# Chrissie-Law/Causal-Domain-Clustering-for-Multi-Domain-Recommendation

Hardware: AMD Instinct MI355X
Metric: train samples/sec + AUC parity, PLE 3-domain batch 4096 at 1/2/4/8 MI355X (higher is better)
Workload: dtype bf16; 1 GPU; PLE 3-domain full training step (fwd + BCE + whole-table L2 + bwd + Adam), 26 fields x vocab 1000000, emb_dim=16, batch 4096/GPU; global_batch=4096, table_mode=lazy, hip_graph=True, row_sort_one_batch_ahead=True, id_dist=uniform, parallelism=dp1, attention_branch=False, full=False, steady_state=True, preroll_steps=1785, flush_every=64

## Files before the change

causal-domain-clustering-for-multi-domain-recommendation_amd/csrc/embedding.hip:

```cpp
#include "common.h"
#include "adam_dense.h"

template <int VEC>
__global__ void __launch_bounds__(256) k_gather_fwd(const int32_t* __restrict__ ids, const int32_t* __restrict__ offsets,
                                                    const float* __restrict__ table, float* __restrict__ out,
                                                    __bf16* __restrict__ out_h, int64_t ld_out_h,
                                                    int32_t* __restrict__ idx_out, int32_t* __restrict__ err_flag,
                                                    int64_t n_pos, int32_t F, int32_t D, int64_t R) {
    CDC_PRIO_MAIN();
    const int chunks = D / VEC;
    const int64_t total = n_pos * chunks;
    for (int64_t i = (int64_t)blockIdx.x * blockDim.x + threadIdx.x; i < total; i += (int64_t)gridDim.x * blockDim.x) {
        const int64_t pos = i / chunks;
        const int c = (int)(i - pos * chunks);
        const int f = (int)(pos % F);
        const int32_t row = (int32_t)((uint32_t)ids[pos] + (uint32_t)offsets[f]);
        const bool ok = row >= 0 && (int64_t)row < R;
        if (c == 0 && idx_out) idx_out[pos] = ok ? row : -1;
        if (!ok && c == 0 && err_flag) atomicMax(err_flag, (int32_t)(pos < 0x7ffffffe ? pos + 1 : 0x7fffffff));
        if (VEC == 4) {
            float4 val = make_float4(0.f, 0.f, 0.f, 0.f);
            if (ok) val = *reinterpret_cast<const float4*>(table + (int64_t)row * D + c * 4);
            *reinterpret_cast<float4*>(out + pos * D + c * 4) = val;
            if (out_h) {
                typedef __bf16 h4_t __attribute__((ext_vector_type(4)));
                h4_t h = {(__bf16)val.x, (__bf16)val.y, (__bf16)val.z, (__bf16)val.w};
                *reinterpret_cast<h4_t*>(out_h + (pos / F) * ld_out_h + (int64_t)f * D + c * 4) = h;
            }
        } else {
            const float v = ok ? table[(int64_t)row * D + c] : 0.f;
            out[pos * D + c] = v;
            if (out_h) out_h[(pos / F) * ld_out_h + (int64_t)f * D + c] = (__bf16)v;
        }
    }
}

extern "C" int cdc_embed_gather_fwd(const int32_t* ids, const int32_t* offsets, const float* table, float* out,
                                    int32_t* idx_out, int32_t* err_flag, int64_t B, int32_t F, int32_t D, int64_t R,
                                    void* stream) {
    return cdc_embed_gather_fwd_h(ids, offsets, table, out, nullptr, 0, idx_out, err_flag, B, F, D, R, stream);
}
extern "C" int cdc_embed_gather_fwd_h(const int32_t* ids, const int32_t* offsets, const float* table, float* out, void* out_h_,
                                      int64_t ld_out_h, int32_t* idx_out, int32_t* err_flag, int64_t B, int32_t F, int32_t D, int64_t R,
                                      void* stream) {
    __bf16* out_h = reinterpret_cast<__bf16*>(out_h_);
    CDC_CHECK_ARG(ids && offsets && table && out, CDC_E_BADARG, "embed_gather_fwd: null pointer");
    CDC_CHECK_ARG(!out_h || (ld_out_h >= (int64_t)F * D && (((uintptr_t)out_h) & 7) == 0 && ld_out_h % 4 == 0), CDC_E_BADARG,
                  "embed_gather_fwd: malformed bf16 shadow");
    CDC_CHECK_ARG(B >= 0 && F > 0 && D > 0 && R > 0, CDC_E_BADARG, "embed_gather_fwd: bad sizes B=%ld F=%d D=%d R=%ld",
                  (long)B, F, D, (long)R);
    if (B == 0) return 0;
    const int64_t n_pos = B * F;
    const bool vec = (D % 4 == 0) && (((uintptr_t)table | (uintptr_t)out) % 16 == 0);
    const int64_t total = n_pos * (vec ? D / 4 : D);
    int blocks = (int)std::min<int64_t>(cdc_ceil_div(total, 256), 256 * 16);
    if (vec)
        hipLaunchKernelGGL(k_gather_fwd<4>, dim3(blocks), dim3(256), 0, (hipStream_t)stream, ids, offsets, table, out, out_h, ld_out_h,
                           idx_out, err_flag, n_pos, F, D, R);
    else
        hipLaunchKernelGGL(k_gather_fwd<1>, dim3(blocks), dim3(256), 0, (hipStream_t)stream, ids, offsets, table, out, out_h, ld_out_h,
                           idx_out, err_flag, n_pos, F, D, R);
    CDC_LAUNCH_CHECK("embed_gather_fwd");
    return 0;
}

__global__ void __launch_bounds__(256) k_embed_index(const int32_t* __restrict__ ids, const int32_t* __restrict__ offsets,
                                                     int32_t* __restrict__ idx_out, int32_t* __restrict__ err_flag, int64_t n_pos,
                                                     int32_t F, int64_t R) {
    for (int64_t pos = (int64_t)blockIdx.x * blockDim.x + threadIdx.x; pos < n_pos; pos += (int64_t)gridDim.x * blockDim.x) {
        const int32_t row = (int32_t)((uint32_t)ids[pos] + (uint32_t)offsets[pos % F]);
        const bool ok = row >= 0 && (int64_t)row < R;
        if (!ok && err_flag) atomicMax(err_flag, (int32_t)(pos < 0x7ffffffe ? pos + 1 : 0x7fffffff));
        idx_out[pos] = ok ? row : -1;
    }
}
extern "C" int cdc_embed_index(const int32_t* ids, const int32_t* offsets, int32_t* idx_out, int32_t* err_flag, int64_t B, int32_t F,
                               int64_t R, void* stream) {
    CDC_CHECK_ARG(ids && offsets && idx_out && B > 0 && F > 0 && R > 0, CDC_E_BADARG, "embed_index: bad argument");
    int blocks = (int)std::min<int64_t>(cdc_ceil_div(B * F, 256), 4096);
    hipLaunchKernelGGL(k_embed_index, dim3(blocks), dim3(256), 0, (hipStream_t)stream, ids, offsets, idx_out, err_flag, B * F, F, R);
    CDC_LAUNCH_CHECK("embed_index");
    return 0;
}

#define SORT_THREADS 1024
#define SORT_CHUNK CDC_SORT_MAX_B

__device__ __forceinline__ void lds_bitonic_sort(uint64_t* keys, int n_pad, int tid) {
    for (int k = 2; k <= n_pad; k <<= 1) {
        for (int j = k >> 1; j > 0; j >>= 1) {
            for (int t = tid; t < (n_pad >> 1); t += SORT_THREADS) {
                const int lo = ((t & ~(j - 1)) << 1) | (t & (j - 1));
                const int hi = lo | j;
                const bool up = (lo & k) == 0;
                const uint64_t a = keys[lo], b = keys[hi];
                if ((a > b) == up) { keys[lo] = b; keys[hi] = a; }
            }
            const int next_j = j > 1 ? (j >> 1) : k;
            if (j >= 64 || next_j >= 64) __syncthreads();
            else {
                __builtin_amdgcn_fence(__ATOMIC_SEQ_CST, "wavefront");
                __builtin_amdgcn_wave_barrier();
            }
        }
    }
    __syncthreads();
}

__device__ __forceinline__ int block_exclusive_scan(int v, int32_t* wave_tot, int tid, int& total) {
    const int lane = tid & 63, wave = tid >> 6;
    int inc = v;
#pragma unroll
    for (int off = 1; off < 64; off <<= 1) {
        const int t = __shfl_up(inc, off, 64);
        if (lane >= off) inc += t;
    }
    if (lane == 63) wave_tot[wave] = inc;
    __syncthreads();
    int base = 0, all = 0;
#pragma unroll
    for (int w = 0; w < SORT_THREADS / 64; ++w) {
        const int t = wave_tot[w];
        base += (w < wave) ? t : 0;
        all += t;
    }
    __syncthreads();
    total = all;
    return base + inc - v;
}

__device__ __forceinline__ void dedupe_sorted(const uint64_t* keys, int n, int32_t* scan, int32_t* __restrict__ urow,
                                              int32_t* __restrict__ sst, int32_t* __restrict__ prm, int32_t* __restrict__ cnt_out,
                                              int tid) {
    const int per = (n + SORT_THREADS - 1) / SORT_THREADS;
    const int begin = tid * per;
    int local = 0;
    for (int i = begin; i < begin + per && i < n; ++i) {
        const bool head = (i == 0) || ((keys[i] >> 32) != (keys[i - 1] >> 32));
        local += head ? 1 : 0;
    }
    int total;
    int u = block_exclusive_scan(local, scan, tid, total);
    for (int i = begin; i < begin + per && i < n; ++i) {
        const uint64_t k = keys[i];
        const bool head = (i == 0) || ((k >> 32) != (keys[i - 1] >> 32));
        if (head) {
            urow[u] = (int32_t)(uint32_t)(k >> 32);
            sst[u] = i;
            ++u;
        }
        prm[i] = (int32_t)(uint32_t)k;
    }
    if (tid == 0) {
        sst[total] = n;
        *cnt_out = total;
    }
}

struct SortSrc {
    const int32_t* idx;
    const int32_t* offsets;
    int64_t R;
    int32_t* step;
    double* acc;
    int32_t n_acc;
    int32_t* err_flag;
};
__device__ __forceinline__ uint32_t sort_row(const SortSrc& s, int64_t i, int f, int F) {
    const int32_t v = s.idx[i * F + f];
    if (!s.offsets) return (uint32_t)v;
    const int32_t row = (int32_t)((uint32_t)v + (uint32_t)s.offsets[f]);
    if (row >= 0 && (int64_t)row < s.R) return (uint32_t)row;
    if (s.err_flag) {
        const int64_t pos = i * F + f;
        atomicMax(s.err_flag, (int32_t)(pos < 0x7ffffffe ? pos + 1 : 0x7fffffff));
    }
    return 0xffffffffu;
}
__device__ __forceinline__ void sort_begin_step(const SortSrc& s, int tid) {
    if (s.step && blockIdx.x == 0 && blockIdx.y == 0) {
        if (tid == 0) *s.step += 1;
        if (tid < s.n_acc) s.acc[tid] = 0.0;
    }
}

__global__ void __launch_bounds__(SORT_THREADS) k_sort_dedupe(const SortSrc src, int32_t* __restrict__ uniq_row,
                                                              int32_t* __restrict__ seg_start, int32_t* __restrict__ perm,
                                                              int32_t* __restrict__ uniq_cnt, int32_t B, int32_t F,
                                                              int32_t n_pad) {
    extern __shared__ __attribute__((aligned(16))) unsigned char smem_raw[];
    uint64_t* keys = reinterpret_cast<uint64_t*>(smem_raw);
    int32_t* scan = reinterpret_cast<int32_t*>(keys + n_pad);
    const int f = blockIdx.x;
    const int tid = threadIdx.x;
    for (int i = tid; i < n_pad; i += SORT_THREADS) {
        uint64_t k = ~0ull;
        if (i < B) k = ((uint64_t)sort_row(src, i, f, F) << 32) | (uint32_t)i;
        keys[i] = k;
    }
    sort_begin_step(src, tid);
    __syncthreads();
    lds_bitonic_sort(keys, n_pad, tid);
    dedupe_sorted(keys, B, scan, uniq_row + (int64_t)f * B, seg_start + (int64_t)f * (B + 1), perm + (int64_t)f * B, uniq_cnt + f, tid);
}

__global__ void __launch_bounds__(SORT_THREADS) k_sort_chunk(const SortSrc src, uint64_t* __restrict__ runs, int32_t B,
                                                             int32_t F, int32_t chunk) {
    extern __shared__ __attribute__((aligned(16))) unsigned char smem_raw[];
    uint64_t* keys = reinterpret_cast<uint64_t*>(smem_raw);
    const int f = blockIdx.x, c = blockIdx.y, tid = threadIdx.x;
    const int r0 = c * chunk;
    const int n = min(chunk, B - r0);
    for (int i = tid; i < chunk; i += SORT_THREADS) {
        uint64_t k = ~0ull;
        if (i < n) k = ((uint64_t)sort_row(src, r0 + i, f, F) << 32) | (uint32_t)(r0 + i);
        keys[i] = k;
    }
    sort_begin_step(src, tid);
    __syncthreads();
    lds_bitonic_sort(keys, chunk, tid);
    uint64_t* out = runs + (int64_t)f * B + r0;
    for (int i = tid; i < n; i += SORT_THREADS) out[i] = keys[i];
}
__device__ __forceinline__ int group_sum(int v, int P) {
    for (int off = 1; off < P; off <<= 1) v += __shfl_xor(v, off, 64);
    return v;
}
__global__ void __launch_bounds__(256) k_merge_runs(const uint64_t* __restrict__ runs, uint64_t* __restrict__ merged, int32_t B,
                                                    int32_t F, int32_t chunk, int32_t n_runs, int32_t P) {
    const int64_t t = (int64_t)blockIdx.x * blockDim.x + threadIdx.x;
    const int64_t item = t / P;
    const int q = (int)(t - item * P);
    const bool valid = item < (int64_t)F * B;
    const int f = valid ? (int)(item / B) : 0;
    const int i = valid ? (int)(item - (int64_t)f * B) : 0;
    const uint64_t* a = runs + (int64_t)f * B;
    const uint64_t key = a[i];
    const int r = i / chunk;
    int lo = 0;
    if (valid && q < n_runs) {
        if (q == r) lo = i - r * chunk;
        else {
            const uint64_t* other = a + (int64_t)q * chunk;
            int hi = min(chunk, B - q * chunk);
            while (lo < hi) {
                const int mid = (lo + hi) >> 1;
                if (other[mid] < key) lo = mid + 1; else hi = mid;
            }
        }
    }
    const int pos = group_sum(lo, P);
    if (valid && q == 0) merged[(int64_t)f * B + pos] = key;
}
template <typename K, bool IDX>
__global__ void __launch_bounds__(SORT_THREADS) k_merge_lds(const void* __restrict__ src, uint64_t* __restrict__ merged, int32_t B,
                                                            int32_t F, int32_t n_runs, int32_t run_len, int32_t P) {
    extern __shared__ __attribute__((aligned(16))) unsigned char smem_raw[];
    K* keys = reinterpret_cast<K*>(smem_raw);
    const int f = blockIdx.x, r = blockIdx.y, tid = threadIdx.x;
    if (IDX) {
        const int32_t* idx = static_cast<const int32_t*>(src);
        for (int i = tid; i < B; i += SORT_THREADS) keys[i] = (K)(uint32_t)idx[(int64_t)i * F + f];
    } else {
        const uint64_t* a = static_cast<const uint64_t*>(src) + (int64_t)f * B;
        for (int i = tid; i < B; i += SORT_THREADS) keys[i] = (K)a[i];
    }
    __syncthreads();
    const int base = r * run_len;
    const int n_r = min(run_len, B - base);
    const int rounds = (n_r * P + SORT_THREADS - 1) / SORT_THREADS;
    for (int it = 0; it < rounds; ++it) {
        const int t = it * SORT_THREADS + tid;
        const int item = t / P, q = t - item * P;
        const bool valid = item < n_r;
        const K key = keys[valid ? base + item : base];
        int lo = 0;
        if (valid && q < n_runs) {
            if (q == r) lo = item;
            else {
                const K* other = keys + q * run_len;
                int hi = min(run_len, B - q * run_len);
                if (IDX && q < r) { while (lo < hi) { const int mid = (lo + hi) >> 1; if (other[mid] <= key) lo = mid + 1; else hi = mid; } }
                else              { while (lo < hi) { const int mid = (lo + hi) >> 1; if (other[mid] <  key) lo = mid + 1; else hi = mid; } }
            }
        }
        const int pos = group_sum(lo, P);
        if (valid && q == 0)
            merged[(int64_t)f * B + pos] = IDX ? (((uint64_t)key << 32) | (uint32_t)(base + item)) : (uint64_t)key;
    }
}
#define MERGE_LDS_MAX (144 * 1024)
__global__ void __launch_bounds__(SORT_THREADS) k_dedupe_merged(const uint64_t* __restrict__ merged, int32_t* __restrict__ uniq_row,
                                                                int32_t* __restrict__ seg_start, int32_t* __restrict__ perm,
                                                                int32_t* __restrict__ uniq_cnt, int32_t B, int32_t F) {
    __shared__ int32_t scan[SORT_THREADS];
    const int f = blockIdx.x;
    dedupe_sorted(merged + (int64_t)f * B, B, scan, uniq_row + (int64_t)f * B, seg_start + (int64_t)f * (B + 1), perm + (int64_t)f * B,
                  uniq_cnt + f, threadIdx.x);
}

static int sort_dedupe_launch(const SortSrc& src, int32_t* uniq_row, int32_t* seg_start, int32_t* perm, int32_t* uniq_cnt,
                              uint64_t* scratch, int64_t B, int32_t F, void* stream) {
    const int32_t* idx = src.idx;
    CDC_CHECK_ARG(idx && uniq_row && seg_start && perm && uniq_cnt, CDC_E_BADARG, "embed_sort_dedupe: null pointer");
    CDC_CHECK_ARG(B > 0 && F > 0, CDC_E_BADARG, "embed_sort_dedupe: bad sizes");
    CDC_CHECK_ARG(B <= CDC_SORT_MAX_ROWS, CDC_E_TOOBIG, "embed_sort_dedupe: B=%ld exceeds %d", (long)B, CDC_SORT_MAX_ROWS);
    CDC_CHECK_ARG(scratch || B <= SORT_CHUNK, CDC_E_BADARG, "embed_sort_dedupe: B > %d needs a scratch buffer of 2*F*B uint64", SORT_CHUNK);
    static bool attr_set = false;
    if (!attr_set) {
        hipError_t e = hipFuncSetAttribute((const void*)k_sort_dedupe, hipFuncAttributeMaxDynamicSharedMemorySize, 160 * 1024);
        if (e == hipSuccess) e = hipFuncSetAttribute((const void*)k_sort_chunk, hipFuncAttributeMaxDynamicSharedMemorySize, 160 * 1024);
        if (e == hipSuccess) e = hipFuncSetAttribute((const void*)k_merge_lds<uint64_t, false>, hipFuncAttributeMaxDynamicSharedMemorySize, 160 * 1024);
        if (e != hipSuccess) { cdc_set_error("embed_sort_dedupe: cannot raise LDS limit: %s", hipGetErrorString(e)); return (int)e; }
        attr_set = true;
    }
    hipStream_t st = (hipStream_t)stream;
    if (B <= 1024 || (!scratch && B <= SORT_CHUNK)) {
        int n_pad = SORT_THREADS;
        while (n_pad < B) n_pad <<= 1;
        const size_t lds = (size_t)n_pad * 8 + SORT_THREADS * 4;
        hipLaunchKernelGGL(k_sort_dedupe, dim3(F), dim3(SORT_THREADS), lds, st, src, uniq_row, seg_start, perm, uniq_cnt, (int32_t)B, F, n_pad);
        CDC_LAUNCH_CHECK("embed_sort_dedupe");
        return 0;
    }
    int chunk = 512;
    while (chunk < SORT_CHUNK && (int64_t)chunk * 8 < B) chunk <<= 1;
    const int n_runs = (int)cdc_ceil_div(B, chunk);
    uint64_t* runs = scratch;
    uint64_t* merged = scratch + (int64_t)F * B;
    hipLaunchKernelGGL(k_sort_chunk, dim3(F, n_runs), dim3(SORT_THREADS), (size_t)chunk * 8, st, src, runs, (int32_t)B, F, chunk);
    CDC_LAUNCH_CHECK("embed_sort_chunk");
    int P = 1;
    while (P < n_runs) P <<= 1;
    CDC_CHECK_ARG(P <= 64, CDC_E_TOOBIG, "embed_sort_dedupe: %d runs", n_runs);
    if ((size_t)B * 8 <= MERGE_LDS_MAX) {
        hipLaunchKernelGGL((k_merge_lds<uint64_t, false>), dim3(F, n_runs), dim3(SORT_THREADS), (size_t)B * 8, st, runs, merged, (int32_t)B, F,
                           n_runs, chunk, P);
    } else {
        const int64_t blocks = cdc_ceil_div((int64_t)F * B * P, 256);
        hipLaunchKernelGGL(k_merge_runs, dim3((unsigned)blocks), dim3(256), 0, st, runs, merged, (int32_t)B, F, chunk, n_runs, P);
    }
    CDC_LAUNCH_CHECK("embed_merge_runs");
    hipLaunchKernelGGL(k_dedupe_merged, dim3(F), dim3(SORT_THREADS), 0, st, merged, uniq_row, seg_start, perm, uniq_cnt, (int32_t)B, F);
    CDC_LAUNCH_CHECK("embed_dedupe_merged");
    return 0;
}

extern "C" int cdc_embed_sort_dedupe(const int32_t* idx, int32_t* uniq_row, int32_t* seg_start, int32_t* perm,
                                     int32_t* uniq_cnt, uint64_t* scratch, int64_t B, int32_t F, void* stream) {
    const SortSrc src = {idx, nullptr, 0, nullptr, nullptr, 0, nullptr};
    return sort_dedupe_launch(src, uniq_row, seg_start, perm, uniq_cnt, scratch, B, F, stream);
}
extern "C" int cdc_embed_sort_dedupe_ids(const int32_t* ids, const int32_t* offsets, int64_t R, int32_t* step_dev, double* accumulators,
                                         int32_t n_acc, int32_t* err_flag, int32_t* uniq_row, int32_t* seg_start, int32_t* perm,
                                         int32_t* uniq_cnt, uint64_t* scratch, int64_t B, int32_t F, void* stream) {
    CDC_CHECK_ARG(offsets && R > 0 && n_acc >= 0 && n_acc <= 64 && (n_acc == 0 || accumulators) && (step_dev || n_acc == 0), CDC_E_BADARG,
                  "embed_sort_dedupe_ids: bad argument");
    const SortSrc src = {ids, offsets, R, step_dev, accumulators, n_acc, err_flag};
    return sort_dedupe_launch(src, uniq_row, seg_start, perm, uniq_cnt, scratch, B, F, stream);
}

__global__ void __launch_bounds__(256) k_merge_n(const int32_t* __restrict__ idx, uint64_t* __restrict__ merged, int32_t B, int32_t F,
                                                 int32_t n_runs, int32_t run_len, int32_t P) {
    const int64_t t = (int64_t)blockIdx.x * blockDim.x + threadIdx.x;
    const int64_t item = t / P;
    const int q = (int)(t - item * P);
    const bool valid = item < (int64_t)F * B;
    const int f = valid ? (int)(item / B) : 0;
    const int i = valid ? (int)(item - (int64_t)f * B) : 0;
    const uint32_t row = (uint32_t)idx[(int64_t)i * F + f];
    const int r = i / run_len;
    int lo = 0;
    if (valid && q < n_runs) {
        if (q == r) lo = i - r * run_len;
        else {
            const int32_t* col = idx + (int64_t)q * run_len * F + f;
            int hi = run_len;
            if (q < r) { while (lo < hi) { const int mid = (lo + hi) >> 1; if ((uint32_t)col[(int64_t)mid * F] <= row) lo = mid + 1; else hi = mid; } }
            else       { while (lo < hi) { const int mid = (lo + hi) >> 1; if ((uint32_t)col[(int64_t)mid * F] <  row) lo = mid + 1; else hi = mid; } }
        }
    }
    const int pos = group_sum(lo, P);
    if (valid && q == 0) merged[(int64_t)f * B + pos] = ((uint64_t)row << 32) | (uint32_t)i;
}
extern "C" int cdc_embed_merge_dedupe(const int32_t* idx, int32_t* uniq_row, int32_t* seg_start, int32_t* perm, int32_t* uniq_cnt,
                                      uint64_t* scratch, int64_t B, int32_t F, int32_t n_runs, void* stream) {
    CDC_CHECK_ARG(idx && uniq_row && seg_start && perm && uniq_cnt && scratch, CDC_E_BADARG, "embed_merge_dedupe: null pointer");
    CDC_CHECK_ARG(B > 0 && F > 0 && n_runs > 0 && B % n_runs == 0, CDC_E_BADARG, "embed_merge_dedupe: bad sizes");
    CDC_CHECK_ARG(B <= CDC_SORT_MAX_ROWS, CDC_E_TOOBIG, "embed_merge_dedupe: B=%ld exceeds %d", (long)B, CDC_SORT_MAX_ROWS);
    hipStream_t st = (hipStream_t)stream;
    int P = 1;
    while (P < n_runs) P <<= 1;
    CDC_CHECK_ARG(P <= 64, CDC_E_TOOBIG, "embed_merge_dedupe: %d runs", n_runs);
    static bool attr_set = false;
    if (!attr_set) {
        hipError_t e = hipFuncSetAttribute((const void*)k_merge_lds<uint32_t, true>, hipFuncAttributeMaxDynamicSharedMemorySize, 160 * 1024);
        if (e != hipSuccess) { cdc_set_error("embed_merge_dedupe: cannot raise LDS limit: %s", hipGetErrorString(e)); return (int)e; }
        attr_set = true;
    }
    if ((size_t)B * 4 <= MERGE_LDS_MAX) {
        hipLaunchKernelGGL((k_merge_lds<uint32_t, true>), dim3(F, n_runs), dim3(SORT_THREADS), (size_t)B * 4, st, idx, scratch, (int32_t)B, F,
                           n_runs, (int32_t)(B / n_runs), P);
    } else {
        const int64_t blocks = cdc_ceil_div((int64_t)F * B * P, 256);
        hipLaunchKernelGGL(k_merge_n, dim3((unsigned)blocks), dim3(256), 0, st, idx, scratch, (int32_t)B, F, n_runs, (int32_t)(B / n_runs), P);
    }
    CDC_LAUNCH_CHECK("embed_merge_n");
    hipLaunchKernelGGL(k_dedupe_merged, dim3(F), dim3(SORT_THREADS), 0, st, scratch, uniq_row, seg_start, perm, uniq_cnt, (int32_t)B, F);
    CDC_LAUNCH_CHECK("embed_dedupe_merged");
    return 0;
}

#define SEG_SPLIT 64
#define SEG_DIRECT 8
#define SEG_BLOCK 512
#define SEG_LONG_BLOCKS 64
#define SEG_LIST_CAP (CDC_SORT_MAX_ROWS / SEG_LONG_BLOCKS)

struct SegSink {
    float* rowgrad;
    float* w; float* m; float* v;
    int32_t* last;
    const int32_t* uniq_row;
    AdamConsts c;
    float step_size, bc2s;
    int32_t t;
};
template <int VEC>
__device__ __forceinline__ void seg_finish(const SegSink& k, int64_t slot, int D, int d0, const float (&acc)[VEC]) {
    if (!k.w) {
        float* dst = k.rowgrad + slot * D + d0;
        if (VEC == 4) *reinterpret_cast<float4*>(dst) = make_float4(acc[0], acc[1 % VEC], acc[2 % VEC], acc[3 % VEC]);
        else dst[0] = acc[0];
        return;
    }
    const int64_t row = k.uniq_row[slot];
    if (row < 0) return;
    const int64_t e0 = row * D + d0;
    float wv[VEC], mv[VEC], vv[VEC];
    if (VEC == 4) {
        const float4 a4 = *reinterpret_cast<const float4*>(k.w + e0), b4 = *reinterpret_cast<const float4*>(k.m + e0),
                     c4 = *reinterpret_cast<const float4*>(k.v + e0);
        wv[0] = a4.x; wv[1 % VEC] = a4.y; wv[2 % VEC] = a4.z; wv[3 % VEC] = a4.w;
        mv[0] = b4.x; mv[1 % VEC] = b4.y; mv[2 % VEC] = b4.z; mv[3 % VEC] = b4.w;
        vv[0] = c4.x; vv[1 % VEC] = c4.y; vv[2 % VEC] = c4.z; vv[3 % VEC] = c4.w;
    } else {
        wv[0] = k.w[e0]; mv[0] = k.m[e0]; vv[0] = k.v[e0];
    }
#pragma unroll
    for (int q = 0; q < VEC; ++q) adam_elem(wv[q], mv[q], vv[q], acc[q], k.c, k.step_size, k.bc2s);
    if (VEC == 4) {
        *reinterpret_cast<float4*>(k.w + e0) = make_float4(wv[0], wv[1 % VEC], wv[2 % VEC], wv[3 % VEC]);
        *reinterpret_cast<float4*>(k.m + e0) = make_float4(mv[0], mv[1 % VEC], mv[2 % VEC], mv[3 % VEC]);
        *reinterpret_cast<float4*>(k.v + e0) = make_float4(vv[0], vv[1 % VEC], vv[2 % VEC], vv[3 % VEC]);
    } else {
        k.w[e0] = wv[0]; k.m[e0] = mv[0]; k.v[e0] = vv[0];
    }
    if (d0 == 0) k.last[row] = k.t;
}
__device__ __forceinline__ SegSink seg_sink_store(float* rowgrad) {
    SegSink k = {};
    k.rowgrad = rowgrad;
    return k;
}

template <int VEC>
__device__ __forceinline__ void seg_direct_body(int bid, int nblocks, const float* __restrict__ d_out, const int32_t* __restrict__ seg_start,
                                                const int32_t* __restrict__ perm, const int32_t* __restrict__ uniq_cnt,
                                                const int32_t* __restrict__ uniq_row, const SegSink& sink,
                                                int32_t B, int32_t F, int32_t D, int32_t max_len) {
    const int chunks = D / VEC;
    const int64_t total = (int64_t)F * B * chunks;
    for (int64_t i = (int64_t)bid * blockDim.x + threadIdx.x; i < total; i += (int64_t)nblocks * blockDim.x) {
        const int c = (int)(i % chunks);
        const int64_t slot = i / chunks;
        const int f = (int)(slot / B);
        const int j = (int)(slot - (int64_t)f * B);
        if (j >= uniq_cnt[f]) continue;
        if (uniq_row && uniq_row[slot] < 0) continue;
        const int32_t* sst = seg_start + (int64_t)f * (B + 1);
        const int32_t* prm = perm + (int64_t)f * B;
        const int k0 = sst[j], k1 = sst[j + 1];
        if (max_len > 0 && k1 - k0 >= max_len) continue;
        float acc[VEC];
#pragma unroll
        for (int q = 0; q < VEC; ++q) acc[q] = 0.f;
        for (int k = k0; k < k1; k += 8) {
            int p[8];
            float v[8][VEC];
#pragma unroll
            for (int q = 0; q < 8; ++q) p[q] = (k + q < k1) ? prm[k + q] : -1;
#pragma unroll
            for (int q = 0; q < 8; ++q) {
                const float* src = d_out + ((int64_t)(p[q] >= 0 ? p[q] : 0) * F + f) * D + c * VEC;
                if (p[q] >= 0) {
                    if (VEC == 4) {
                        const float4 t = *reinterpret_cast<const float4*>(src);
                        v[q][0] = t.x; v[q][1] = t.y; v[q][2] = t.z; v[q][3] = t.w;
                    } else {
                        v[q][0] = src[0];
                    }
                }
            }
#pragma unroll
            for (int q = 0; q < 8; ++q)
                if (p[q] >= 0) {
#pragma unroll
                    for (int e = 0; e < VEC; ++e) acc[e] = __fadd_rn(acc[e], v[q][e]);
                }
        }
        seg_finish<VEC>(sink, slot, D, c * VEC, acc);
    }
}
template <int VEC>
__global__ void __launch_bounds__(256) k_segment_sum_direct(const float* __restrict__ d_out, const int32_t* __restrict__ seg_start,
                                                            const int32_t* __restrict__ perm, const int32_t* __restrict__ uniq_cnt,
                                                            const int32_t* __restrict__ uniq_row, float* __restrict__ rowgrad,
                                                            int32_t B, int32_t F, int32_t D, int32_t max_len) {
    seg_direct_body<VEC>(blockIdx.x, gridDim.x, d_out, seg_start, perm, uniq_cnt, uniq_row, seg_sink_store(rowgrad), B, F, D, max_len);
}
extern "C" int cdc_embed_segment_sum_direct(const float* d_out, const int32_t* seg_start, const int32_t* perm,
                                            const int32_t* uniq_cnt, const int32_t* uniq_row, float* rowgrad, int64_t B, int32_t F,
                                            int32_t D, void* stream) {
    CDC_CHECK_ARG(d_out && seg_start && perm && uniq_cnt && rowgrad, CDC_E_BADARG, "embed_segment_sum_direct: null pointer");
    CDC_CHECK_ARG(B > 0 && F > 0 && D > 0 && B <= CDC_SORT_MAX_ROWS, CDC_E_BADARG, "embed_segment_sum_direct: bad sizes");
    const bool vec = (D % 4 == 0) && (((uintptr_t)d_out | (uintptr_t)rowgrad) % 16 == 0);
    int blocks = (int)std::min<int64_t>(cdc_ceil_div((int64_t)F * B * (vec ? D / 4 : D), 256), 8192);
    if (vec)
        hipLaunchKernelGGL(k_segment_sum_direct<4>, dim3(blocks), dim3(256), 0, (hipStream_t)stream, d_out, seg_start, perm, uniq_cnt, uniq_row,
                           rowgrad, (int32_t)B, F, D, 0);
    else
        hipLaunchKernelGGL(k_segment_sum_direct<1>, dim3(blocks), dim3(256), 0, (hipStream_t)stream, d_out, seg_start, perm, uniq_cnt, uniq_row,
                           rowgrad, (int32_t)B, F, D, 0);
    CDC_LAUNCH_CHECK("embed_segment_sum_direct");
    return 0;
}

template <int BATCH = 16>
__device__ __forceinline__ float seg_serial_sum(const float* __restrict__ d_out, const int32_t* __restrict__ prm, int begin, int end,
                                                int F, int D, int f, int d) {
    float acc = 0.f;
    for (int k = begin; k < end; k += BATCH) {
        int p[BATCH];
        float x[BATCH];
#pragma unroll
        for (int q = 0; q < BATCH; ++q) p[q] = (k + q < end) ? prm[k + q] : -1;
#pragma unroll
        for (int q = 0; q < BATCH; ++q) x[q] = p[q] >= 0 ? d_out[((int64_t)p[q] * F + f) * D + d] : 0.f;
#pragma unroll
        for (int q = 0; q < BATCH; ++q)
            if (p[q] >= 0) acc = __fadd_rn(acc, x[q]);
    }
    return acc;
}
template <int VEC>
__device__ __forceinline__ void seg_long_body(int f, int by, const float* __restrict__ d_out, const int32_t* __restrict__ seg_start,
                                              const int32_t* __restrict__ perm, const int32_t* __restrict__ uniq_cnt,
                                              const SegSink& sink, int32_t B, int32_t F, int32_t D, int32_t subs,
                                              int32_t min_len) {
    __shared__ int32_t list[SEG_LIST_CAP];
    __shared__ int32_t n_list;
    __shared__ __attribute__((aligned(16))) float parts[256 * VEC];
    const int tid = threadIdx.x, lane = tid & 63, wave = tid >> 6;
    const int n = uniq_cnt[f];
    const int32_t* sst = seg_start + (int64_t)f * (B + 1);
    const int32_t* prm = perm + (int64_t)f * B;
    if (tid == 0) n_list = 0;
    __syncthreads();
    for (int j = by + SEG_LONG_BLOCKS * tid; j < n; j += SEG_LONG_BLOCKS * 256)
        if (sst[j + 1] - sst[j] >= min_len) list[atomicAdd(&n_list, 1)] = j;
    __syncthreads();
    const int count = n_list;
    if (count == 0) return;
    const bool block_rows = subs > 1;
    for (int i = wave; i < count; i += 4) {
        const int j = list[i];
        const int k0 = sst[j], len = sst[j + 1] - k0;
        if (block_rows && len >= SEG_BLOCK) continue;
        const int64_t slot = (int64_t)f * B + j;
        if (subs <= 1) {
            for (int d = lane; d < D; d += 64) {
                const float one[1] = {seg_serial_sum(d_out, prm + k0, 0, len, F, D, f, d)};
                seg_finish<1>(sink, slot, D, d, one);
            }
            continue;
        }
        const int sub = lane / D, d = lane - sub * D;
        const bool split = len >= SEG_SPLIT;
        int begin = 0, end = (sub == 0) ? len : 0;
        if (split) {
            const int q = (len + subs - 1) / subs;
            begin = min(sub * q, len);
            end = min(begin + q, len);
        }
        float acc = seg_serial_sum(d_out, prm + k0, begin, end, F, D, f, d);
        if (split) {
            float total = __shfl(acc, d, 64);
            for (int s2 = 1; s2 < subs; ++s2) total = __fadd_rn(total, __shfl(acc, s2 * D + d, 64));
            acc = total;
        }
        if (sub == 0) {
            const float one[1] = {acc};
            seg_finish<1>(sink, slot, D, d, one);
        }
    }
    if (!block_rows) return;
    const int chunks = D / VEC;
    const int P = 256 / chunks;
    const int part = tid / chunks, d = (tid - part * chunks) * VEC;
    for (int i = 0; i < count; ++i) {
        const int j = list[i];
        const int k0 = sst[j], len = sst[j + 1] - k0;
        if (len < SEG_BLOCK) continue;
        const int q = (len + P - 1) / P;
        const int begin = min(part * q, len), end = min(begin + q, len);
        float acc[VEC];
#pragma unroll
        for (int e = 0; e < VEC; ++e) acc[e] = 0.f;
        if (part < P) {
// ... 943 lines not shown
```

Baseline: 13.11 million samples/s.

## Add register-resident bitonic sort-dedupe kernel for mid-size batches

Adds a single-kernel sort-and-dedupe path for batches between SORT_THREADS and four keys per thread. Each thread keeps four keys in registers, and the bitonic network exchanges partners with DPP or shuffles inside a wave and through LDS across waves. When a field's row range is narrow, keys are packed into 32 bits (relative row plus 12-bit position) to halve exchange traffic. This replaces the chunk-sort plus multi-pass merge launches for batch 4096 and so cuts launches and global scratch traffic. The cost is more register pressure and only one block per field, which limits parallelism to F blocks.

```diff
diff --git a/causal-domain-clustering-for-multi-domain-recommendation_amd/csrc/embedding.hip b/causal-domain-clustering-for-multi-domain-recommendation_amd/csrc/embedding.hip
--- a/causal-domain-clustering-for-multi-domain-recommendation_amd/csrc/embedding.hip
+++ b/causal-domain-clustering-for-multi-domain-recommendation_amd/csrc/embedding.hip
@@ -204,6 +204,164 @@
     dedupe_sorted(keys, B, scan, uniq_row + (int64_t)f * B, seg_start + (int64_t)f * (B + 1), perm + (int64_t)f * B, uniq_cnt + f, tid);
 }
 
+#define SORT_REG_KPT 4
+#define SORT_REG_N (SORT_THREADS * SORT_REG_KPT)
+#define SORT_REG_POS_BITS 12
+#define SORT_REG_BAD_REL ((1u << (32 - SORT_REG_POS_BITS)) - 1u)
+static_assert((1 << SORT_REG_POS_BITS) == SORT_REG_N, "the position field holds every position of the network");
+template <typename K>
+__device__ __forceinline__ void sort_cmpx(K& a, K& b, bool up) {
+    const bool swap = (b < a) == up;
+    const K x = a, y = b;
+    a = swap ? y : x;
+    b = swap ? x : y;
+}
+__device__ __forceinline__ uint32_t lane_xor(uint32_t v, int m) {
+    switch (m) {
+    case 1: return (uint32_t)__builtin_amdgcn_update_dpp(0, (int)v, 0xB1, 0xf, 0xf, false);
+    case 2: return (uint32_t)__builtin_amdgcn_update_dpp(0, (int)v, 0x4E, 0xf, 0xf, false);
+    case 8: return (uint32_t)__builtin_amdgcn_update_dpp(0, (int)v, 0x128, 0xf, 0xf, false);
+    default: return (uint32_t)__shfl_xor((int)v, m, 64);
+    }
+}
+__device__ __forceinline__ uint64_t lane_xor(uint64_t v, int m) {
+    return ((uint64_t)lane_xor((uint32_t)(v >> 32), m) << 32) | lane_xor((uint32_t)v, m);
+}
+template <typename K>
+__device__ __forceinline__ void sort_reg_network(K (&k)[SORT_REG_KPT], K* xch, int tid) {
+    sort_cmpx(k[0], k[1], true);
+    sort_cmpx(k[2], k[3], false);
+#pragma unroll
+    for (int kk = 4; kk <= SORT_REG_N; kk <<= 1) {
+        const bool up = (tid & (kk >> 2)) == 0;
+#pragma unroll
+        for (int j = kk >> 1; j >= SORT_REG_KPT; j >>= 1) {
+            const int tj = j >> 2;
+            const bool keep_min = ((tid & tj) == 0) == up;
+            K o[SORT_REG_KPT];
+            if (tj >= 64) {
+                __syncthreads();
+#pragma unroll
+                for (int r = 0; r < SORT_REG_KPT; ++r) xch[r * SORT_THREADS + tid] = k[r];
+                __syncthreads();
+#pragma unroll
+                for (int r = 0; r < SORT_REG_KPT; ++r) o[r] = xch[r * SORT_THREADS + (tid ^ tj)];
+            } else {
+#pragma unroll
+                for (int r = 0; r < SORT_REG_KPT; ++r) o[r] = lane_xor(k[r], tj);
+            }
+#pragma unroll
+            for (int r = 0; r < SORT_REG_KPT; ++r) k[r] = ((o[r] < k[r]) == keep_min) ? o[r] : k[r];
+        }
+        sort_cmpx(k[0], k[2], up);
+        sort_cmpx(k[1], k[3], up);
+        sort_cmpx(k[0], k[1], up);
+        sort_cmpx(k[2], k[3], up);
+    }
+}
+__global__ void __launch_bounds__(SORT_THREADS) k_sort_dedupe_reg(const SortSrc src, int32_t* __restrict__ uniq_row,
+                                                                  int32_t* __restrict__ seg_start, int32_t* __restrict__ perm,
+                                                                  int32_t* __restrict__ uniq_cnt, int32_t B, int32_t F) {
+    __shared__ __attribute__((aligned(16))) uint64_t xch[SORT_REG_N];
+    uint32_t* xw = reinterpret_cast<uint32_t*>(xch);
+    const int f = blockIdx.x, tid = threadIdx.x, lane = tid & 63, wave = tid >> 6;
+    uint32_t row[SORT_REG_KPT], pos[SORT_REG_KPT];
+    uint32_t rmin = 0xffffffffu, rmax = 0u;
+#pragma unroll
+    for (int r = 0; r < SORT_REG_KPT; ++r) {
+        pos[r] = r * SORT_THREADS + tid;
+        row[r] = 0xffffffffu;
+        if ((int)pos[r] < B) row[r] = sort_row(src, pos[r], f, F);
+        if (row[r] != 0xffffffffu) {
+            rmin = min(rmin, row[r]);
+            rmax = max(rmax, row[r]);
+        }
+    }
+    sort_begin_step(src, tid);
+#pragma unroll
+    for (int off = 1; off < 64; off <<= 1) {
+        rmin = min(rmin, lane_xor(rmin, off));
+        rmax = max(rmax, lane_xor(rmax, off));
+    }
+    if (lane == 0) {
+        xw[wave] = rmin;
+        xw[SORT_THREADS / 64 + wave] = rmax;
+    }
+    __syncthreads();
+#pragma unroll
+    for (int w = 0; w < SORT_THREADS / 64; ++w) {
+        rmin = min(rmin, xw[w]);
+        rmax = max(rmax, xw[SORT_THREADS / 64 + w]);
+    }
+    if (rmin > rmax) rmin = rmax = 0u;
+    const bool narrow = rmax - rmin < SORT_REG_BAD_REL;
+    __syncthreads();
+    if (narrow) {
+        uint32_t k[SORT_REG_KPT];
+#pragma unroll
+        for (int r = 0; r < SORT_REG_KPT; ++r) {
+            const uint32_t rel = row[r] == 0xffffffffu ? SORT_REG_BAD_REL : row[r] - rmin;
+            k[r] = (int)pos[r] < B ? ((rel << SORT_REG_POS_BITS) | pos[r]) : 0xffffffffu;
+        }
+        sort_reg_network(k, xw, tid);
+#pragma unroll
+        for (int r = 0; r < SORT_REG_KPT; ++r) {
+            const uint32_t rel = k[r] >> SORT_REG_POS_BITS;
+            row[r] = rel == SORT_REG_BAD_REL ? 0xffffffffu : rmin + rel;
+            pos[r] = k[r] & (SORT_REG_N - 1);
+        }
+    } else {
+        uint64_t k[SORT_REG_KPT];
+#pragma unroll
+        for (int r = 0; r < SORT_REG_KPT; ++r) k[r] = (int)pos[r] < B ? (((uint64_t)row[r] << 32) | pos[r]) : ~0ull;
+        sort_reg_network(k, xch, tid);
+#pragma unroll
+        for (int r = 0; r < SORT_REG_KPT; ++r) {
+            row[r] = (uint32_t)(k[r] >> 32);
+            pos[r] = (uint32_t)k[r];
+        }
+    }
+    uint32_t* last_row = xw;
+    int32_t* wave_tot = reinterpret_cast<int32_t*>(xw) + SORT_THREADS;
+    __syncthreads();
+    last_row[tid] = row[SORT_REG_KPT - 1];
+    __syncthreads();
+    uint32_t prev = tid > 0 ? last_row[tid - 1] : 0u;
+    const int e0 = tid * SORT_REG_KPT;
+    bool head[SORT_REG_KPT];
+    int local = 0;
+#pragma unroll
+    for (int r = 0; r < SORT_REG_KPT; ++r) {
+        head[r] = (e0 + r < B) && (e0 + r == 0 || row[r] != prev);
+        local += head[r] ? 1 : 0;
+        prev = row[r];
+    }
+    int total;
+    int u = block_exclusive_scan(local, wave_tot, tid, total);
+    int32_t* urow = uniq_row + (int64_t)f * B;
+    int32_t* sst = seg_start + (int64_t)f * (B + 1);
+    int32_t* prm = perm + (int64_t)f * B;
+#pragma unroll
+    for (int r = 0; r < SORT_REG_KPT; ++r) {
+        if (head[r]) {
+            urow[u] = (int32_t)row[r];
+            sst[u] = e0 + r;
+            ++u;
+        }
+    }
+    if (e0 + SORT_REG_KPT <= B && (reinterpret_cast<uintptr_t>(prm + e0) & 15) == 0) {
+        *reinterpret_cast<int4*>(prm + e0) = make_int4((int32_t)pos[0], (int32_t)pos[1], (int32_t)pos[2], (int32_t)pos[3]);
+    } else {
+#pragma unroll
+        for (int r = 0; r < SORT_REG_KPT; ++r)
+            if (e0 + r < B) prm[e0 + r] = (int32_t)pos[r];
+    }
+    if (tid == 0) {
+        sst[total] = B;
+        uniq_cnt[f] = total;
+    }
+}
+
 __global__ void __launch_bounds__(SORT_THREADS) k_sort_chunk(const SortSrc src, uint64_t* __restrict__ runs, int32_t B,
                                                              int32_t F, int32_t chunk) {
     extern __shared__ __attribute__((aligned(16))) unsigned char smem_raw[];
@@ -315,6 +473,11 @@
         attr_set = true;
     }
     hipStream_t st = (hipStream_t)stream;
+    if (B > SORT_THREADS && B <= SORT_REG_N) {
+        hipLaunchKernelGGL(k_sort_dedupe_reg, dim3(F), dim3(SORT_THREADS), 0, st, src, uniq_row, seg_start, perm, uniq_cnt, (int32_t)B, F);
+        CDC_LAUNCH_CHECK("embed_sort_dedupe_reg");
+        return 0;
+    }
     if (B <= 1024 || (!scratch && B <= SORT_CHUNK)) {
         int n_pad = SORT_THREADS;
         while (n_pad < B) n_pad <<= 1;
```

Result: faster. 13.39 million samples/s (median of 6 runs) (+2.2%).

## Add single-block LDS radix sort-dedupe for mid-size embedding batches

Applied to the files above, without the earlier changes.

Adds a per-field block radix sort (8-bit digits, ballot-based ranking) that sorts row ids and positions in LDS and dedupes in one kernel for batches between 1024 and 4096. It skips digit passes whose bits are identical across all keys. This replaces the chunked bitonic sort plus multi-pass merge path, which needs a scratch buffer and several launches at batch 4096. In exchange it adds a new code path with its own register pressure and LDS layout, and it limits parallelism to one block per field.

```diff
diff --git a/causal-domain-clustering-for-multi-domain-recommendation_amd/csrc/embedding.hip b/causal-domain-clustering-for-multi-domain-recommendation_amd/csrc/embedding.hip
--- a/causal-domain-clustering-for-multi-domain-recommendation_amd/csrc/embedding.hip
+++ b/causal-domain-clustering-for-multi-domain-recommendation_amd/csrc/embedding.hip
@@ -204,6 +204,146 @@
     dedupe_sorted(keys, B, scan, uniq_row + (int64_t)f * B, seg_start + (int64_t)f * (B + 1), perm + (int64_t)f * B, uniq_cnt + f, tid);
 }
 
+#define SORT_RADIX_MAX 4096
+#define SORT_RADIX_ITEMS (SORT_RADIX_MAX / SORT_THREADS)
+#define SORT_WAVES (SORT_THREADS / 64)
+__global__ void __launch_bounds__(SORT_THREADS) k_sort_dedupe_radix(const SortSrc src, int32_t* __restrict__ uniq_row,
+                                                                    int32_t* __restrict__ seg_start, int32_t* __restrict__ perm,
+                                                                    int32_t* __restrict__ uniq_cnt, int32_t B, int32_t F) {
+    __shared__ uint32_t rows[SORT_RADIX_MAX];
+    __shared__ uint32_t pos[SORT_RADIX_MAX];
+    __shared__ int32_t hist[SORT_WAVES * 256];
+    __shared__ int32_t wave_tot[SORT_RADIX_ITEMS * SORT_WAVES];
+    __shared__ uint32_t red_or[SORT_WAVES], red_and[SORT_WAVES];
+    const int f = blockIdx.x;
+    const int tid = threadIdx.x, lane = tid & 63, wave = tid >> 6;
+    if (B > SORT_RADIX_MAX) return;
+    const int rounds = (B + SORT_THREADS - 1) / SORT_THREADS;
+
+    uint32_t any = 0u, all = ~0u;
+#pragma unroll
+    for (int r = 0; r < SORT_RADIX_ITEMS; ++r) {
+        const int i = r * SORT_THREADS + tid;
+        if (r < rounds) {
+            uint32_t k = ~0u;
+            if (i < B) {
+                k = sort_row(src, i, f, F);
+                any |= k;
+                all &= k;
+            }
+            rows[i] = k;
+            pos[i] = (uint32_t)i;
+        }
+    }
+    sort_begin_step(src, tid);
+#pragma unroll
+    for (int off = 32; off > 0; off >>= 1) {
+        any |= (uint32_t)__shfl_xor((int)any, off, 64);
+        all &= (uint32_t)__shfl_xor((int)all, off, 64);
+    }
+    if (lane == 0) { red_or[wave] = any; red_and[wave] = all; }
+    __syncthreads();
+    any = 0u; all = ~0u;
+#pragma unroll
+    for (int w = 0; w < SORT_WAVES; ++w) { any |= red_or[w]; all &= red_and[w]; }
+    const uint32_t differ = any ^ all;
+
+    const int per_wave = rounds * 64;
+    const uint64_t lanes_below = (1ull << lane) - 1ull;
+    for (int shift = 0; shift < 32; shift += 8) {
+        if (((differ >> shift) & 0xffu) == 0u) continue;
+#pragma unroll
+        for (int j = 0; j < 4; ++j) hist[wave * 256 + j * 64 + lane] = 0;
+        __builtin_amdgcn_fence(__ATOMIC_SEQ_CST, "wavefront");
+        __builtin_amdgcn_wave_barrier();
+        uint32_t k[SORT_RADIX_ITEMS], v[SORT_RADIX_ITEMS];
+        int rk[SORT_RADIX_ITEMS];
+#pragma unroll
+        for (int r = 0; r < SORT_RADIX_ITEMS; ++r) {
+            k[r] = 0u; v[r] = 0u; rk[r] = 0;
+            if (r < rounds) {
+                const int i = wave * per_wave + r * 64 + lane;
+                k[r] = rows[i];
+                v[r] = pos[i];
+                const uint32_t d = (k[r] >> shift) & 0xffu;
+                uint64_t peers = ~0ull;
+#pragma unroll
+                for (int b = 0; b < 8; ++b) {
+                    const bool bit = (d >> b) & 1u;
+                    const uint64_t m = __ballot(bit);
+                    peers &= bit ? m : ~m;
+                }
+                const int before = __popcll(peers & lanes_below);
+                int old = 0;
+                if (before == 0) old = atomicAdd(&hist[wave * 256 + (int)d], (int)__popcll(peers));
+                rk[r] = __shfl(old, __ffsll((unsigned long long)peers) - 1, 64) + before;
+            }
+        }
+        __syncthreads();
+        {
+            const int d = tid >> 2, w0 = (tid & 3) * 4;
+            int h[4], sum = 0;
+#pragma unroll
+            for (int j = 0; j < 4; ++j) { h[j] = hist[(w0 + j) * 256 + d]; sum += h[j]; }
+            int total;
+            int run = block_exclusive_scan(sum, wave_tot, tid, total);
+#pragma unroll
+            for (int j = 0; j < 4; ++j) { hist[(w0 + j) * 256 + d] = run; run += h[j]; }
+        }
+        __syncthreads();
+#pragma unroll
+        for (int r = 0; r < SORT_RADIX_ITEMS; ++r) {
+            if (r < rounds) {
+                const int dst = hist[wave * 256 + (int)((k[r] >> shift) & 0xffu)] + rk[r];
+                rows[dst] = k[r];
+                pos[dst] = v[r];
+            }
+        }
+        __syncthreads();
+    }
+
+    bool head[SORT_RADIX_ITEMS];
+    uint64_t hmask[SORT_RADIX_ITEMS];
+#pragma unroll
+    for (int r = 0; r < SORT_RADIX_ITEMS; ++r) {
+        const int i = r * SORT_THREADS + tid;
+        head[r] = (r < rounds) && (i < B) && (i == 0 || rows[i] != rows[i - 1]);
+        hmask[r] = __ballot(head[r]);
+        if (lane == 0) wave_tot[r * SORT_WAVES + wave] = (int)__popcll(hmask[r]);
+    }
+    __syncthreads();
+    int inc = wave_tot[lane];
+    const int own = inc;
+#pragma unroll
+    for (int off = 1; off < 64; off <<= 1) {
+        const int t = __shfl_up(inc, off, 64);
+        if (lane >= off) inc += t;
+    }
+    const int total = __shfl(inc, 63, 64);
+    const int excl = inc - own;
+    int32_t* urow = uniq_row + (int64_t)f * B;
+    int32_t* sst = seg_start + (int64_t)f * (B + 1);
+    int32_t* prm = perm + (int64_t)f * B;
+#pragma unroll
+    for (int r = 0; r < SORT_RADIX_ITEMS; ++r) {
+        const int i = r * SORT_THREADS + tid;
+        const int base = __shfl(excl, r * SORT_WAVES + wave, 64);
+        if (r < rounds && i < B) {
+            if (head[r]) {
+                const int u = base + (int)__popcll(hmask[r] & lanes_below);
+                urow[u] = (int32_t)rows[i];
+                sst[u] = i;
+            }
+            prm[i] = (int32_t)pos[i];
+        }
+    }
+    if (tid == 0) {
+        sst[total] = B;
+        uniq_cnt[f] = total;
+    }
+}
+static_assert(SORT_RADIX_ITEMS * SORT_WAVES == 64, "the dedupe scans its (round, wave) head counts inside one wave");
+
 __global__ void __launch_bounds__(SORT_THREADS) k_sort_chunk(const SortSrc src, uint64_t* __restrict__ runs, int32_t B,
                                                              int32_t F, int32_t chunk) {
     extern __shared__ __attribute__((aligned(16))) unsigned char smem_raw[];
@@ -315,6 +455,11 @@
         attr_set = true;
     }
     hipStream_t st = (hipStream_t)stream;
+    if (B > 1024 && B <= SORT_RADIX_MAX) {
+        hipLaunchKernelGGL(k_sort_dedupe_radix, dim3(F), dim3(SORT_THREADS), 0, st, src, uniq_row, seg_start, perm, uniq_cnt, (int32_t)B, F);
+        CDC_LAUNCH_CHECK("embed_sort_dedupe_radix");
+        return 0;
+    }
     if (B <= 1024 || (!scratch && B <= SORT_CHUNK)) {
         int n_pad = SORT_THREADS;
         while (n_pad < B) n_pad <<= 1;
```

Result: faster. 13.35 million samples/s before, 13.55 million samples/s after (median of 6 runs) (+1.5%).
